# marcros/PartsBasedDetector

Measured on AMD Instinct MI355X. Metric: detections/sec (whole node), person model @640×480, 1/2/4/8 MI355X, higher is better.
Workload: dtype f32

## Files before the change

### partsbaseddetector_amd/csrc/pbd_kernels_dp.hip

```cpp
#include "pbd_device.h"
#include "pbd_dp.h"

#include <math.h>

#include <algorithm>

namespace pbd {

#ifdef PBD_DT_STATS
__device__ unsigned long long g_dt_stats[16];
#define DT_STAT(i)                                                                                      \
    do {                                                                                                \
        const unsigned long long m_ = __ballot(1);                                                      \
        if ((int)__lane_id() == __ffsll((long long)m_) - 1) {                                           \
            atomicAdd(&g_dt_stats[2 * (i)], 1ull);                                                      \
            atomicAdd(&g_dt_stats[2 * (i) + 1], (unsigned long long)__popcll(m_));                      \
        }                                                                                               \
    } while (0)
#else
#define DT_STAT(i)
#endif

template <typename R, bool BZ>
__device__ __forceinline__ R quad_isect(double a, double b, int x0, int x1, R y0f, R y1f)
{
    const double y0 = (double)y0f, y1 = (double)y1f;
    const int dx = x1 - x0;
    const double dd = (double)dx;
    const double sq = (double)(int)__umul24((unsigned)dx, (unsigned)(x1 + x0));
    const double num = BZ ? (y1 - y0) + a * sq : ((y1 - y0) - b * dd) + a * sq;
    return (R)(num / ((2 * a) * dd));
}
template <typename R, bool BZ>
__device__ __forceinline__ R quad_val(double a, double b, int x, R y)
{
    if (BZ) return (R)(a * (double)__mul24(x, x) + (double)y);
    return (R)((a * (double)__mul24(x, x) + b * (double)x) + (double)y);
}

template <typename R> struct StkPairT { R sa, sb, za; unsigned vv; };
static_assert(sizeof(StkPairT<float>) == kStkPairF32 && sizeof(StkPairT<double>) == kStkPairF64, "host sizes the spill stack with these");

#ifndef PBD_DT_CH
#define PBD_DT_CH 16
#endif
constexpr int kDtCH = PBD_DT_CH;
#ifndef PBD_DT_CHC
#define PBD_DT_CHC 16
#endif
constexpr int kDtCHC = PBD_DT_CHC;
#ifndef PBD_DT_RING
#define PBD_DT_RING 8
#endif
constexpr int kDtT = PBD_DT_RING;

template <typename R, bool NARROW>
struct DtRing {
    static constexpr int kSlotBytes = 64 * (2 * (int)sizeof(R) + 4);
    char *zs;
    char *vp;
    StkPairT<R> *g;
    double a, b;
    int lo;
    int tmask, sbytes, soff;
    __device__ __forceinline__ int T() const { return NARROW ? tmask + 1 : kDtT; }
    __device__ __forceinline__ int slot_of(int idx) const { return NARROW ? (idx & tmask) : (idx & (kDtT - 1)); }
    __device__ __forceinline__ int off(int slot) const { return NARROW ? slot * sbytes : slot * kSlotBytes; }
    __device__ __forceinline__ R &z(int slot) { return *reinterpret_cast<R *>(zs + off(slot)); }
    __device__ __forceinline__ R &s(int slot) { return *reinterpret_cast<R *>(zs + off(slot) + (NARROW ? soff : 64 * (int)sizeof(R))); }
    __device__ __forceinline__ int &v(int slot) { return *reinterpret_cast<int *>(vp + off(slot)); }
    __device__ __forceinline__ void push_below(int idx, R zk, R sk, int vk)
    {
        const int slot = slot_of(idx);
        if (idx - lo >= T()) {
            DT_STAT(3);
            const int sl = slot_of(lo);
            g[(size_t)(lo >> 1) * 64] = StkPairT<R>{s(sl), s(sl + 1), z(sl), (unsigned)v(sl) | ((unsigned)v(sl + 1) << 16)};
            lo += 2;
        }
        z(slot) = zk; s(slot) = sk; v(slot) = vk;
    }
    template <bool BZ>
    __device__ __forceinline__ void pop(int idx, R &zk, R &sk, int &vk)
    {
        const int slot = slot_of(idx);
        zk = z(slot); sk = s(slot); vk = v(slot);
        asm volatile("" : "+v"(zk), "+v"(sk), "+v"(vk));
        if (idx < lo) {
            DT_STAT(4);
            const StkPairT<R> e = g[(size_t)((lo - 2) >> 1) * 64];
            const int va = (int)(e.vv & 0xffffu), vb = (int)(e.vv >> 16);
            const int sl = slot_of(lo - 2);
            z(sl) = e.za; s(sl) = e.sa; v(sl) = va;
            sk = e.sb; vk = vb;
            zk = BZ ? quad_isect<R, true>(a, b, va, vb, e.sa, e.sb) : quad_isect<R, false>(a, b, va, vb, e.sa, e.sb);
            lo -= 2;
        }
    }
    static __device__ __forceinline__ DtRing make(char *smem, int lanep, int sh, StkPairT<R> *g, double a, double b)
    {
        const int L = NARROW ? (64 >> sh) : 64;
        return DtRing{smem + lanep * (int)sizeof(R), smem + 2 * L * (int)sizeof(R) + lanep * 4, g, a, b, 0,
                      (kDtT << (NARROW ? sh : 0)) - 1, L * (2 * (int)sizeof(R) + 4), L * (int)sizeof(R)};
    }
};

template <int EPW> __device__ __forceinline__ int dt_get(const int *w, int i)
{
    constexpr int BITS = 32 / EPW;
    return EPW == 1 ? w[i] : (int)(((unsigned)w[i / EPW] >> (BITS * (i % EPW))) & ((1u << BITS) - 1u));
}
template <int EPW> __device__ __forceinline__ void dt_put(int *w, int i, int v)
{
    constexpr int BITS = 32 / EPW;
    if (EPW == 1) w[i] = v;
    else w[i / EPW] |= v << (BITS * (i % EPW));
}

template <typename R, bool BZ, int CH, int EPW, bool NARROW, class LoadChunk, class StoreChunk>
__device__ __forceinline__ void dt_stream(int N, double a, double b, int os0, DtRing<R, NARROW> ring, LoadChunk load, StoreChunk store)
{
    R cur[CH], nxt[CH];
    load(0, cur);
    int k = 0, vk = 0;
    R zk = -RealLimits<R>::inf(), sk = cur[0];
    ring.lo = 0;
    for (int q0 = 0; q0 < N; q0 += CH) {
        if (q0 + CH < N) load(q0 + CH, nxt);
#pragma unroll
        for (int i = 0; i < CH; ++i) {
            const int q = q0 + i;
            if (q >= 1 && q < N) {
                const R sq = cur[i];
                DT_STAT(0);
                R s = quad_isect<R, BZ>(a, b, vk, q, sk, sq);
                while (s <= zk && k > 0) {
                    DT_STAT(1);
                    --k;
                    ring.template pop<BZ>(k, zk, sk, vk);
                    s = quad_isect<R, BZ>(a, b, vk, q, sk, sq);
                }
                ring.push_below(k, zk, sk, vk);
                ++k;
                vk = q; zk = s; sk = sq;
            }
        }
#pragma unroll
        for (int i = 0; i < CH; ++i) cur[i] = nxt[i];
    }
    const int nch = (N + CH - 1) / CH;
    constexpr int NW = CH / EPW;
    for (int cidx = nch - 1; cidx >= 0; --cidx) {
        const int q0 = cidx * CH;
        R out[CH];
        int ptr[NW];
#pragma unroll
        for (int i = 0; i < NW; ++i) ptr[i] = 0;
#pragma unroll
        for (int i = CH - 1; i >= 0; --i) {
            out[i] = (R)0;
            const int q = q0 + i;
            if (q < N) {
                const R osf = (R)(os0 + q);
                DT_STAT(5);
                while (!(zk < osf)) {
                    DT_STAT(2);
                    --k;
                    ring.template pop<BZ>(k, zk, sk, vk);
                }
                out[i] = quad_val<R, BZ>(a, b, os0 + q - vk, sk);
                dt_put<EPW>(ptr, i, vk);
            }
        }
        store(q0, out, ptr);
    }
}

typedef float v4f_u __attribute__((ext_vector_type(4), aligned(4)));
typedef _Float16 v8h_u __attribute__((ext_vector_type(8), aligned(2)));
static_assert(kDtCHC % 8 == 0 && kDtCH % 8 == 0, "int16 pointers and fp16 responses are read 8 at a time");

template <typename R, typename PT> struct DtLine {
    ScoreSrc<R> src;
    int N;
    R *outv; PT *outp;
    int ostr;
    double a, b;
    int os;
    size_t stk;
};
template <typename R, bool RH, typename PT, bool COLS>
__device__ __forceinline__ DtLine<R, PT> dt_line(const DpParams &p, int flat, int j, int fl)
{
    const int l = (COLS ? p.col2level : p.row2level)[flat];
    const LevelDesc d = p.lv[l];
    const int idx = flat - (COLS ? p.coloff : p.rowoff)[l];
    const DtJob job = p.jobs[j];
    const LevelPlanes<DpParams> pl(p, d, p.frame0 + fl, fl);
    const size_t jo = (size_t)j * pl.HW, go = (size_t)job.gm * pl.HW;
    const size_t stk = (size_t)(fl * p.JG + j) * p.stk_per_jf;
    if (COLS) return {{pl.tmp<R>(jo + (size_t)idx * d.rows), nullptr}, d.rows, pl.dt<R>(jo + idx), pl.iy<PT>(go + idx), d.cols,
                      job.ay, job.by, job.osy, stk};
    return {pl.score<R>(job.from_acc, RH, job.plane, (size_t)idx * d.cols), d.cols, pl.tmp<R>(jo + idx), pl.ix<PT>(go + idx), d.rows,
            job.ax, job.bx, job.osx, stk};
}

template <typename R, int CH>
__device__ __forceinline__ void dt_load_chunk(const ScoreSrc<R> &src, int N, int q0, R *buf)
{
    if (src.h) {
        if (q0 + CH <= N) {
#pragma unroll
            for (int v = 0; v < CH / 8; ++v) {
                const v8h_u a0 = *reinterpret_cast<const v8h_u *>(src.h + q0 + 8 * v);
#pragma unroll
                for (int e = 0; e < 8; ++e) buf[8 * v + e] = (R)(float)a0[e];
            }
        } else {
#pragma unroll
            for (int i = 0; i < CH; ++i) buf[i] = (q0 + i < N) ? (R)(float)src.h[q0 + i] : (R)0;
        }
    } else if (sizeof(R) == 4 && q0 + CH <= N) {
        const float *srcf = reinterpret_cast<const float *>(src.v);
#pragma unroll
        for (int v = 0; v < CH / 4; ++v) {
            const v4f_u a0 = *reinterpret_cast<const v4f_u *>(srcf + q0 + 4 * v);
            buf[4 * v] = a0.x; buf[4 * v + 1] = a0.y; buf[4 * v + 2] = a0.z; buf[4 * v + 3] = a0.w;
        }
    } else {
#pragma unroll
        for (int i = 0; i < CH; ++i) buf[i] = (q0 + i < N) ? src.v[q0 + i] : (R)0;
    }
}
template <typename R, typename PT, int CH>
__device__ __forceinline__ void dt_store_chunk(const DtLine<R, PT> &ln, int q0, const R *out, const int *ptr)
{
    R *vp = ln.outv + (size_t)q0 * ln.ostr;
    PT *pp = ln.outp + (size_t)q0 * ln.ostr;
#pragma unroll
    for (int i = 0; i < CH; ++i) {
        if (q0 + i < ln.N) { *vp = out[i]; *pp = (PT)dt_get<4 / (int)sizeof(PT)>(ptr, i); }
        vp += ln.ostr; pp += ln.ostr;
    }
}

template <typename R, bool RH, typename PT, bool BZ, bool NARROW, bool COLS>
__global__ __launch_bounds__(64) __attribute__((amdgpu_waves_per_eu(COLS && sizeof(R) == 4 ? (sizeof(PT) == 1 && !NARROW ? 6 : 5) : 1)))
void k_dt_pass(DpParams p)
{
    constexpr int EPW = 4 / (int)sizeof(PT), CH = COLS ? kDtCHC : kDtCH;
    const int sh = p.lane_shift, lanep = threadIdx.x;
    if (lanep >= (64 >> sh)) return;
    const int wv = (int)blockIdx.z >> sh, lane = (((int)blockIdx.z & ((1 << sh) - 1)) << (6 - sh)) + lanep;
    const int flat = wv * 64 + lane;
    if (flat >= (COLS ? p.ncols_flat : p.nrows_flat)) return;
    const DtLine<R, PT> ln = dt_line<R, RH, PT, COLS>(p, flat, blockIdx.x, blockIdx.y);
    __shared__ __attribute__((aligned(16))) char ring_mem[kDtT * DtRing<R, NARROW>::kSlotBytes];
    DtRing<R, NARROW> ring = DtRing<R, NARROW>::make(ring_mem, lanep, sh, reinterpret_cast<StkPairT<R> *>(p.stk) + ln.stk +
                                                                              (COLS ? p.stk_col_off : p.stk_row_off)[wv] + lane, ln.a, ln.b);
    dt_stream<R, BZ, CH, EPW, NARROW>(ln.N, ln.a, ln.b, ln.os, ring,
                                      [&](int q0, R *buf) { dt_load_chunk<R, CH>(ln.src, ln.N, q0, buf); },
                                      [&](int q0, const R *out, const int *ptr) { dt_store_chunk<R, PT, CH>(ln, q0, out, ptr); });
}

static int dt_lane_shift(const DtOptions &o, long long waves64)
{
    if (o.lane_shift >= 0) return o.lane_shift;
    int sh = 0;
    while (sh < 6 && (waves64 << (sh + 1)) <= 6144) ++sh;
    return sh;
}

template <bool COLS> static void launch_dt_coop(const DpParams &p, int coop_g, int nframes, int nflat, bool bz, hipStream_t s);
static bool dt_coop_fits(int longest);
static int dt_coop_min_shift();

template <class F> static void for_flag(bool b, F &&f) { if (b) f(std::true_type{}); else f(std::false_type{}); }
template <class F> static void for_real(bool f64, F &&f) { if (f64) f(double{}); else f(float{}); }
template <class F> static void for_ptr(bool ptr8, F &&f) { if (ptr8) f(uint8_t{}); else f(int16_t{}); }

template <bool COLS>
static void launch_dt_pass(const DpParams &p0, const DtOptions &o, int nframes, bool f64, hipStream_t s)
{
    const int nflat = COLS ? p0.ncols_flat : p0.nrows_flat;
    if (p0.JG == 0 || nflat == 0) return;
    const int nwv = (nflat + 63) / 64;
    DpParams p = p0;
    p.lane_shift = dt_lane_shift(o, (long long)p.JG * nframes * nwv);
    const bool bz = (COLS ? p.bz_y : p.bz_x) != 0, rh = !COLS && !f64 && p.resp_half;
    if (o.coop && p.lane_shift >= dt_coop_min_shift() && !f64 && !rh && p.ptr8 && dt_coop_fits(p.longest)) {
        launch_dt_coop<COLS>(p, o.coop_g, nframes, nflat, bz, s);
        return;
    }
    const dim3 grid(p.JG, nframes, nwv << p.lane_shift);
    for_ptr(p.ptr8 != 0, [&](auto pt) { for_flag(bz, [&](auto z) {
        using PT = decltype(pt);
        constexpr bool BZ = decltype(z)::value;
        if constexpr (!COLS) {
            if (rh) { PBD_LAUNCH((k_dt_pass<float, true, PT, BZ, false, false>), grid, dim3(64), 0, s, p); return; }
        }
        for_real(f64, [&](auto r) { for_flag(p.lane_shift > 0, [&](auto nw) {
            PBD_LAUNCH((k_dt_pass<decltype(r), false, PT, BZ, decltype(nw)::value, COLS>), grid, dim3(64), 0, s, p);
        }); });
    }); });
}
void launch_dt_rows(const DpParams &p, const DtOptions &o, int nframes, bool f64, hipStream_t s) { launch_dt_pass<false>(p, o, nframes, f64, s); }
void launch_dt_cols(const DpParams &p, const DtOptions &o, int nframes, bool f64, hipStream_t s) { launch_dt_pass<true>(p, o, nframes, f64, s); }

template <bool BZ, typename PT, bool COLS, int G>
__global__ __launch_bounds__(64) void k_dt_coop(DpParams p)
{
    constexpr int kCoopRows = G, kCoopW = 64 / G, kCoopLog = (G == 4 ? 4 : 3);
    static_assert(G == 4 || G == 8, "four or eight rows per wave");
    extern __shared__ __attribute__((aligned(16))) char coop_mem[];
    const int lanep = threadIdx.x, grp = lanep >> kCoopLog, sub = lanep & (kCoopW - 1), gl0 = grp << kCoopLog;
    const int nflat = COLS ? p.ncols_flat : p.nrows_flat;
    const int r = (int)blockIdx.z * kCoopRows + grp;
    const bool active = r < nflat;
    const int rr = active ? r : nflat - 1;
    const DtLine<float, PT> ln = dt_line<float, false, PT, COLS>(p, rr, blockIdx.x, blockIdx.y);
    const int N = active ? ln.N : 0, os0 = ln.os, ostr = ln.ostr;
    const double a = ln.a, b = ln.b;
    const float *src = ln.src.v;
    float *outv = ln.outv;
    PT *outp = ln.outp;
    const int maxn = p.longest;
    float *zs = reinterpret_cast<float *>(coop_mem) + (size_t)grp * 3 * maxn, *ys = zs + maxn;
    int *vs = reinterpret_cast<int *>(ys + maxn);
    int nm = N;
#pragma unroll
    for (int o = kCoopW; o < 64; o <<= 1) nm = max(nm, __shfl_xor(nm, o));
    const int Nmax = __builtin_amdgcn_readfirstlane(nm);
    if (Nmax == 0) return;

    float cur = (sub < N) ? src[sub] : 0.0f;
    float ez = -INFINITY, ey = __shfl(cur, gl0);
    int ev = 0, k = 0, wbase = 0;
    if (sub == 0 && N > 0) { zs[0] = ez; ys[0] = ey; vs[0] = 0; }
    for (int q0 = 0; q0 < Nmax; q0 += kCoopW) {
        const float nxt = (q0 + kCoopW + sub < N) ? src[q0 + kCoopW + sub] : 0.0f;
        for (int i = (q0 == 0 ? 1 : 0); i < kCoopW && q0 + i < Nmax; ++i) {
            const int q = q0 + i;
            const bool rowact = q < N;
            const float yq = __shfl(cur, gl0 + i);
            float s;
            unsigned m;
            for (;;) {
                const int e = wbase + sub;
                s = quad_isect<float, BZ>(a, b, ev, q, ey, yq);
                const bool stay = rowact && e <= k && !((s <= ez) && e > 0);
                m = (unsigned)(__ballot(stay) >> gl0) & ((1u << kCoopW) - 1u);
                const bool lower = rowact && m == 0;
                if (!__any(lower)) break;
                if (lower) { wbase -= kCoopW; k = wbase + kCoopW - 1; ez = zs[wbase + sub]; ey = ys[wbase + sub]; ev = vs[wbase + sub]; }
            }
            const int top = wbase + (rowact ? 31 - __clz((int)m) : 0);
            const float snew = __shfl(s, gl0 + (top & (kCoopW - 1)));
            if (rowact) {
                k = top + 1;
                if ((k & (kCoopW - 1)) == 0) wbase = k;
                if (sub == (k & (kCoopW - 1))) { ev = q; ey = yq; ez = snew; zs[k] = snew; ys[k] = yq; vs[k] = q; }
            }
        }
        cur = nxt;
    }
    for (int p0 = 0; p0 < Nmax; p0 += kCoopW) {
        const int pq = p0 + sub;
        const float osf = (float)(os0 + pq);
        int lo = 0, hi = k;
        while (__any(lo < hi)) {
            const int mid = (lo + hi + 1) >> 1;
            const bool lt = zs[mid] < osf;
            if (lo < hi) { if (lt) lo = mid; else hi = mid - 1; }
        }
        if (pq < N) {
            outv[(size_t)pq * ostr] = quad_val<float, BZ>(a, b, os0 + pq - vs[lo], ys[lo]);
            outp[(size_t)pq * ostr] = (PT)vs[lo];
        }
    }
}

static int dt_coop_min_shift() { return 3; }
static bool dt_coop_fits(int longest)
{
    return (size_t)4 * 3 * longest * sizeof(float) <= (size_t)12 * 1024;
}

template <bool COLS, int G>
static void launch_dt_coop_g(const DpParams &p, int nframes, int nflat, bool bz, hipStream_t s)
{
    dim3 grid(p.JG, nframes, (nflat + G - 1) / G);
    const unsigned lds = (unsigned)((size_t)G * 3 * p.longest * sizeof(float));
    if (bz) PBD_LAUNCH((k_dt_coop<true, uint8_t, COLS, G>), grid, dim3(64), lds, s, p);
    else PBD_LAUNCH((k_dt_coop<false, uint8_t, COLS, G>), grid, dim3(64), lds, s, p);
}
template <bool COLS>
static void launch_dt_coop(const DpParams &p, int coop_g, int nframes, int nflat, bool bz, hipStream_t s)
{
    const long long waves4 = (long long)p.JG * nframes * ((nflat + 3) / 4);
    const bool g8 = coop_g ? coop_g == 8 : (waves4 > 6144 && (size_t)8 * 3 * p.longest * sizeof(float) <= (size_t)12 * 1024);
    if (g8) launch_dt_coop_g<COLS, 8>(p, nframes, nflat, bz, s);
    else launch_dt_coop_g<COLS, 4>(p, nframes, nflat, bz, s);
}

template <typename T, int N> struct CellVec;
#define PBD_CELLVEC(T, E, N) template <> struct CellVec<T, N> { typedef E type __attribute__((ext_vector_type(N), aligned(sizeof(E)))); }
PBD_CELLVEC(float, float, 4); PBD_CELLVEC(float, float, 2); PBD_CELLVEC(double, double, 4); PBD_CELLVEC(double, double, 2);
PBD_CELLVEC(int16_t, short, 4); PBD_CELLVEC(int16_t, short, 2); PBD_CELLVEC(uint8_t, unsigned char, 4); PBD_CELLVEC(uint8_t, unsigned char, 2);
PBD_CELLVEC(_Float16, _Float16, 4); PBD_CELLVEC(_Float16, _Float16, 2);
#undef PBD_CELLVEC

template <typename T, int kCpt>
__device__ __forceinline__ void load_cells(const T *src, int n, T *dst)
{
    if (n == kCpt) {
        const typename CellVec<T, kCpt>::type v = *reinterpret_cast<const typename CellVec<T, kCpt>::type *>(src);
#pragma unroll
        for (int e = 0; e < kCpt; ++e) dst[e] = (T)v[e];
    } else {
#pragma unroll
        for (int e = 0; e < kCpt; ++e) dst[e] = (e < n) ? src[e] : (T)0;
    }
}
template <typename T, int kCpt>
__device__ __forceinline__ void load_cells_wide(const T *src, T *dst)
{
    const typename CellVec<T, kCpt>::type v = *reinterpret_cast<const typename CellVec<T, kCpt>::type *>(src);
#pragma unroll
    for (int e = 0; e < kCpt; ++e) dst[e] = (T)v[e];
}
template <typename T, int kCpt>
__device__ __forceinline__ void store_cells(T *dst, int n, const T *src)
{
    if (n == kCpt) {
        typename CellVec<T, kCpt>::type v;
#pragma unroll
        for (int e = 0; e < kCpt; ++e) v[e] = src[e];
        *reinterpret_cast<typename CellVec<T, kCpt>::type *>(dst) = v;
    } else {
#pragma unroll
        for (int e = 0; e < kCpt; ++e) if (e < n) dst[e] = src[e];
    }
}

template <typename R, int kCpt, int MAXM, bool RH>
__global__ __launch_bounds__(256) __attribute__((amdgpu_waves_per_eu(MAXM <= 6 && sizeof(R) == 4 ? 4 : 1)))
void k_dp_combine(DpParams p)
{
    constexpr int SUB = 4 / kCpt;
    const long long gidx = (long long)blockIdx.x * blockDim.x + threadIdx.x;
    const long long qidx = gidx / SUB;
    if (qidx >= p.quad_per_frame) return;
    const int fl = blockIdx.z, frame = p.frame0 + fl;
    const CombineJob cj = p.cjobs[blockIdx.y];
    const LevelDesc d = p.lv[level_of<&LevelDesc::quad_off>(p.lv, 0, p.nlevels, qidx)];
    const int HWi = d.rows * d.cols;
    const size_t HW = (size_t)HWi;
    const int local = (int)(qidx - d.quad_off) * 4 + (int)(gidx % SUB) * kCpt;
    if (local >= HWi) return;
    const int n = min(kCpt, HWi - local);
    const LevelPlanes<DpParams> pl(p, d, frame, fl);
    const R *dtp = pl.dt<R>();
    uint8_t *ik = pl.Ik(local);
    R accv[MAXM][kCpt];
#pragma unroll
    for (int pm = 0; pm < MAXM; ++pm) {
#pragma unroll
        for (int e = 0; e < kCpt; ++e) accv[pm][e] = (R)0;
        if (pm < cj.npar) {
            const ScoreSrc<R> rs = pl.score<R>(false, RH, cj.filter[pm], local);
            if constexpr (RH) {
                _Float16 hv[kCpt];
                load_cells<_Float16, kCpt>(rs.h, n, hv);
#pragma unroll
                for (int e = 0; e < kCpt; ++e) accv[pm][e] = (R)(float)hv[e];
            } else {
                load_cells<R, kCpt>(rs.v, n, accv[pm]);
            }
        }
    }
    const int __attribute__((address_space(4))) *childs = (const int __attribute__((address_space(4))) *)p.childs;
    constexpr int kChildInts = 3 + kMaxMix;
    static_assert(sizeof(ChildDesc) == kChildInts * sizeof(int), "ChildDesc is read as 3 + kMaxMix ints");
    const float __attribute__((address_space(4))) *biasw = (const float __attribute__((address_space(4))) *)p.biasw;
    for (int ch = cj.child_begin; ch < cj.child_end; ++ch) {
        ChildDesc cd;
        {
            const int __attribute__((address_space(4))) *ci = childs + (size_t)ch * kChildInts;
            cd.job_begin = ci[0]; cd.nmix = ci[1]; cd.slot = ci[2];
#pragma unroll
            for (int k = 0; k < MAXM; ++k) cd.bias_off[k] = ci[3 + k];
        }
        const R *dtc = dtp + (size_t)cd.job_begin * HW;
        float bw[MAXM][MAXM];
#pragma unroll
        for (int mm = 0; mm < MAXM; ++mm)
#pragma unroll
            for (int pm = 0; pm < MAXM; ++pm)
                bw[mm][pm] = (mm < cd.nmix && pm < cj.npar) ? biasw[cd.bias_off[mm] + pm] : 0.0f;
        R dtv[MAXM][kCpt];
#pragma unroll
        for (int mm = 0; mm < MAXM; ++mm) {
#pragma unroll
            for (int e = 0; e < kCpt; ++e) dtv[mm][e] = -RealLimits<R>::inf();
            if (mm < cd.nmix) load_cells_wide<R, kCpt>(dtc + (size_t)mm * HW + local, dtv[mm]);
        }
#pragma unroll
        for (int pm = 0; pm < MAXM; ++pm) {
            if (pm < cj.npar) {
                uint8_t oik[kCpt];
                R best[kCpt];
                int bi[kCpt];
#pragma unroll
                for (int e = 0; e < kCpt; ++e) bi[e] = 0;
                if (cd.nmix == 1) {
#pragma unroll
                    for (int e = 0; e < kCpt; ++e) best[e] = dtv[0][e] + (R)bw[0][pm];
                } else {
#pragma unroll
                    for (int e = 0; e < kCpt; ++e) {
                        best[e] = -RealLimits<R>::inf();
#pragma unroll
                        for (int mm = 0; mm < MAXM; ++mm) pick_max<R>(dtv[mm][e] + (R)bw[mm][pm], mm, best[e], bi[e]);
                    }
                }
#pragma unroll
                for (int e = 0; e < kCpt; ++e) {
                    oik[e] = (uint8_t)bi[e];
                    accv[pm][e] = accv[pm][e] + best[e];
                }
                store_cells<uint8_t, kCpt>(ik + (size_t)(cd.slot + pm) * HW, n, oik);
            }
        }
    }
    R *acc = pl.acc<R>(local);
#pragma unroll
    for (int pm = 0; pm < MAXM; ++pm)
        if (pm < cj.npar) store_cells<R, kCpt>(acc + (size_t)(cj.acc_plane + pm) * HW, n, accv[pm]);
}

void launch_dp_combine(const DpParams &p, int ncjobs, int nframes, bool f64, hipStream_t s)
{
    if (ncjobs == 0 || p.quad_per_frame == 0) return;
    const dim3 g2((unsigned)((p.quad_per_frame * 2 + 255) / 256), ncjobs, nframes), g4((unsigned)((p.quad_per_frame + 255) / 256), ncjobs, nframes);
    auto launch = [&](auto m) {
        constexpr int M = decltype(m)::value;
        if (f64) PBD_LAUNCH((k_dp_combine<double, 2, M, false>), g2, dim3(256), 0, s, p);
        else if (p.resp_half) PBD_LAUNCH((k_dp_combine<float, 4, M, true>), g4, dim3(256), 0, s, p);
        else PBD_LAUNCH((k_dp_combine<float, 4, M, false>), g4, dim3(256), 0, s, p);
    };
    if (p.max_mix <= 2) launch(std::integral_constant<int, 2>{});
    else if (p.max_mix <= 4) launch(std::integral_constant<int, 4>{});
    else if (p.max_mix <= 6) launch(std::integral_constant<int, 6>{});
    else if (p.max_mix <= 8) launch(std::integral_constant<int, 8>{});
    else launch(std::integral_constant<int, 16>{});
}

template <typename R>
__global__ __launch_bounds__(256) void k_dp_combine_seq(DpParams p)
{
    const long long idx = (long long)blockIdx.x * blockDim.x + threadIdx.x;
    if (idx >= p.cell_per_frame) return;
    const int fl = blockIdx.z;
    const SeqCombineJob sj = p.sjobs[blockIdx.y];
    const LevelDesc d = p.lv[level_of(p.lv, 0, p.nlevels, idx)];
    const size_t local = (size_t)(idx - d.cell_off);
    const LevelPlanes<DpParams> pl(p, d, p.frame0 + fl, fl);
    const size_t HW = pl.HW;
    const R *dtp = pl.dt<R>((size_t)sj.job_begin * HW + local);
    R dtv[kMaxMix];
    for (int mm = 0; mm < sj.nmix; ++mm) dtv[mm] = dtp[(size_t)mm * HW];
    for (int pm = 0; pm < sj.npar; ++pm) {
        int bi;
        const R best = reduce_max<R>(sj.nmix, [&](int mm) { return dtv[mm] + (R)p.biasw[sj.bias_off[mm] + pm]; }, bi);
        *pl.Ik((size_t)(sj.slot + pm) * HW + local) = (uint8_t)bi;
        R *t = pl.acc<R>((size_t)sj.target[pm] * HW + local);
        const R base = !sj.init[pm] ? *t : pl.score<R>(false, sizeof(R) == 4 && p.resp_half, sj.filter[pm], local)[0];
        *t = base + best;
    }
}

void launch_dp_combine_seq(const DpParams &p, int nsjobs, int nframes, bool f64, hipStream_t s)
{
    if (nsjobs == 0 || p.cell_per_frame == 0) return;
    dim3 grid((unsigned)((p.cell_per_frame + 255) / 256), nsjobs, nframes);
    for_real(f64, [&](auto r) { PBD_LAUNCH(k_dp_combine_seq<decltype(r)>, grid, dim3(256), 0, s, p); });
}

template <typename R>
__global__ __launch_bounds__(256) void k_dp_root(DpParams p)
{
    const long long idx = (long long)blockIdx.x * blockDim.x + threadIdx.x;
    if (idx >= p.cell_per_frame) return;
    const int c = blockIdx.y, fl = blockIdx.z, frame = p.frame0 + fl;
    const RootJob rj = p.rjobs[c];
    const LevelDesc d = p.lv[level_of(p.lv, 0, p.nlevels, idx)];
    const size_t local = (size_t)(idx - d.cell_off);
    const LevelPlanes<DpParams> pl(p, d, frame);
    const bool rh = sizeof(R) == 4 && p.resp_half;
    int bi;
    const R best = reduce_max<R>(rj.nmix, [&](int mm) { return pl.score<R>((rj.from_acc >> mm) & 1, rh, rj.plane[mm], local)[0] + (R)rj.bias; }, bi);
    const size_t o = (size_t)c * pl.HW + local;
    *pl.rootv<R>(o) = best;
    *pl.rooti(o) = bi;
}

void launch_dp_root(const DpParams &p, int nframes, bool f64, hipStream_t s)
{
    if (p.cell_per_frame == 0) return;
    dim3 grid((unsigned)((p.cell_per_frame + 255) / 256), p.NC, nframes);
    for_real(f64, [&](auto r) { PBD_LAUNCH(k_dp_root<decltype(r)>, grid, dim3(256), 0, s, p); });
}

constexpr int kFindEPT = 4, kFindBlock = 256, kFindSpan = kFindEPT * kFindBlock;

template <typename R>
__device__ __forceinline__ int find_hits(const ArgminParams &p, long long base, bool hit[kFindEPT])
{
    const R *rv = static_cast<const R *>(p.rootv);
    int c = 0;
#pragma unroll
    for (int e = 0; e < kFindEPT; ++e) {
        const long long o = base + e;
        hit[e] = o < p.ntotal && rv[o] > (R)p.thresh;
        if (p.root_max) hit[e] = hit[e] && p.root_max[o];
        c += hit[e] ? 1 : 0;
    }
    return c;
}

template <typename R>
__global__ __launch_bounds__(kFindBlock) void k_argmin_count(ArgminParams p)
{
    bool hit[kFindEPT];
    const int c = find_hits<R>(p, (long long)blockIdx.x * kFindSpan + threadIdx.x * kFindEPT, hit);
    __shared__ int wsum[kFindBlock / 64];
    const int lane = threadIdx.x & 63, incl = wave_incl_scan(c);
    if (lane == 63) wsum[threadIdx.x >> 6] = incl;
    __syncthreads();
    if (threadIdx.x == 0) {
        int t = 0;
#pragma unroll
        for (int w = 0; w < kFindBlock / 64; ++w) t += wsum[w];
        p.blk[blockIdx.x] = t;
    }
}

__global__ __launch_bounds__(1024) void k_argmin_scan(ArgminParams p)
{
    __shared__ int wsum[16];
    __shared__ int carry_s;
    if (threadIdx.x == 0) carry_s = 0;
    __syncthreads();
    const int lane = threadIdx.x & 63, w = threadIdx.x >> 6;
    for (int b0 = 0; b0 < p.nblk; b0 += 1024) {
        const int b = b0 + threadIdx.x;
        const int v = b < p.nblk ? p.blk[b] : 0;
        const int incl = wave_incl_scan(v);
        if (lane == 63) wsum[w] = incl;
        __syncthreads();
        int off = carry_s;
        for (int k = 0; k < w; ++k) off += wsum[k];
        if (b < p.nblk) p.blk[b] = off + incl - v;
        __syncthreads();
        if (threadIdx.x == 1023) carry_s = off + incl;
        __syncthreads();
    }
    if (threadIdx.x == 0) p.payload[0] = carry_s;
}

template <typename R>
__global__ __launch_bounds__(kFindBlock) void k_argmin_emit(ArgminParams p)
{
    bool hit[kFindEPT];
    const long long base = (long long)blockIdx.x * kFindSpan + threadIdx.x * kFindEPT;
    const int c = find_hits<R>(p, base, hit);
    __shared__ int wsum[kFindBlock / 64];
    const int lane = threadIdx.x & 63, w = threadIdx.x >> 6, incl = wave_incl_scan(c);
    if (lane == 63) wsum[w] = incl;
    __syncthreads();
    if (c == 0) return;
    int slot = p.blk[blockIdx.x] + incl - c;
    for (int k = 0; k < w; ++k) slot += wsum[k];
    const long long per_frame = p.cell_per_frame * p.NC;
#pragma unroll
    for (int e = 0; e < kFindEPT; ++e) {
        if (!hit[e]) continue;
        const int mine = slot++;
        if (mine >= p.capacity) continue;
        const long long o = base + e;
        const int frame = (int)(o / per_frame);
        root_record(p.payload + 1 + (size_t)mine * p.stride, p.lv, 0, p.nlevels, p.NC, frame, o - (long long)frame * per_frame,
                    static_cast<const R *>(p.rootv)[o], p.rooti[o]);
    }
}

void launch_argmin_find(const ArgminParams &p, bool f64, hipStream_t s)
{
    for_real(f64, [&](auto r) { PBD_LAUNCH(k_argmin_count<decltype(r)>, dim3(p.nblk), dim3(kFindBlock), 0, s, p); });
    PBD_LAUNCH(k_argmin_scan, dim3(1), dim3(1024), 0, s, p);
    for_real(f64, [&](auto r) { PBD_LAUNCH(k_argmin_emit<decltype(r)>, dim3(p.nblk), dim3(kFindBlock), 0, s, p); });
}
int argmin_find_span() { return kFindSpan; }

template <typename R, typename PT>
__global__ __launch_bounds__(64) void k_argmin_walk(ArgminParams p)
{
    __shared__ int visited[kWalkMaxParts][64];
    __shared__ uint8_t visited_m[kWalkMaxParts][64];
    const int ncand = min(p.payload[0], p.capacity);
    for (int i = blockIdx.x * blockDim.x + threadIdx.x; i < ncand; i += gridDim.x * blockDim.x) {
    int32_t *rec = p.payload + 1 + (size_t)i * p.stride;
    const int frame = rec[0], c = rec[1], l = rec[2];
    const LevelDesc d = p.lv[l];
    const LevelPlanes<ArgminParams> pl(p, d, frame);
    const R scale = (R)p.scales[l];
    const PartWalk *walk = p.walk + p.walk_off[c];
    const int nparts = p.walk_off[c + 1] - p.walk_off[c];
    int32_t *rects = rec + 8;
    for (int pidx = 0; pidx < nparts; ++pidx) {
        int x, y, m;
        if (pidx == 0) {
            x = rec[3]; y = rec[4]; m = rec[7];
        } else {
            const PartWalk w = walk[pidx];
            const int par = visited[w.parent][threadIdx.x];
            const WalkPos ch = walk_child<PT>(pl, w, par & 0xffff, par >> 16, visited_m[w.parent][threadIdx.x], p.walk_mode == PBD_WALK_ARGMAX);
            x = ch.x; y = ch.y; m = ch.m;
        }
        visited[pidx][threadIdx.x] = x | (y << 16);
        visited_m[pidx][threadIdx.x] = (uint8_t)m;
        const PartRect r = part_rect<R>(x, y, walk[pidx].ksize[m], scale);
        rects[pidx * 4 + 0] = r.x1;
        rects[pidx * 4 + 1] = r.y1;
        rects[pidx * 4 + 2] = r.x2 - r.x1;
        rects[pidx * 4 + 3] = r.y2 - r.y1;
    }
    rec[0] = frame + p.frame_offset;
    if (p.lv_frame) {
        rec[0] = p.lv_frame[l] + p.frame_offset;
        rec[2] = p.lv_local[l];
    }
    rec[6] = nparts;
    rec[7] = 0;
    }
}

void launch_argmin_walk(const ArgminParams &p, bool f64, hipStream_t s)
{
    const int blocks = std::max(std::min((p.capacity + 63) / 64, 2048), 1);
    for_real(f64, [&](auto r) { for_ptr(p.ptr8 != 0, [&](auto pt) {
        PBD_LAUNCH((k_argmin_walk<decltype(r), decltype(pt)>), dim3(blocks), dim3(64), 0, s, p);
    }); });
}

}

#ifdef PBD_DT_STATS
extern "C" int pbd_debug_dt_stats(unsigned long long *out, int reset)
{
    if (out && hipMemcpyFromSymbol(out, HIP_SYMBOL(pbd::g_dt_stats), sizeof(pbd::g_dt_stats)) != hipSuccess) return -1;
    if (reset) {
        unsigned long long z[16] = {0};
        if (hipMemcpyToSymbol(HIP_SYMBOL(pbd::g_dt_stats), z, sizeof(z)) != hipSuccess) return -1;
    }
    return 0;
}
#endif
```

Before: 1096.

## Batch ring spills and reloads across the wavefront with high/low watermarks

```diff
diff --git a/partsbaseddetector_amd/csrc/pbd_kernels_dp.hip b/partsbaseddetector_amd/csrc/pbd_kernels_dp.hip
--- a/partsbaseddetector_amd/csrc/pbd_kernels_dp.hip
+++ b/partsbaseddetector_amd/csrc/pbd_kernels_dp.hip
@@ -53,6 +53,20 @@
 #define PBD_DT_RING 8
 #endif
 constexpr int kDtT = PBD_DT_RING;
+#ifndef PBD_DT_HIGH
+#define PBD_DT_HIGH 6
+#endif
+#ifndef PBD_DT_LOW
+#define PBD_DT_LOW 2
+#endif
+#ifndef PBD_DT_LOW_RO
+#define PBD_DT_LOW_RO 6
+#endif
+constexpr int kDtHigh = PBD_DT_HIGH;
+constexpr int kDtLow = PBD_DT_LOW;
+constexpr int kDtLowRO = PBD_DT_LOW_RO;
+static_assert(kDtHigh >= 3 && kDtHigh <= kDtT + 1, "a spilling lane has its oldest pair in the ring; a lane over the ring always spills");
+static_assert(kDtLow <= kDtT - 2 && kDtLowRO <= kDtT - 2, "a pair is only reloaded into a ring with room for two entries");
 
 template <typename R, bool NARROW>
 struct DtRing {
@@ -69,16 +83,38 @@
     __device__ __forceinline__ R &z(int slot) { return *reinterpret_cast<R *>(zs + off(slot)); }
     __device__ __forceinline__ R &s(int slot) { return *reinterpret_cast<R *>(zs + off(slot) + (NARROW ? soff : 64 * (int)sizeof(R))); }
     __device__ __forceinline__ int &v(int slot) { return *reinterpret_cast<int *>(vp + off(slot)); }
+    __device__ __forceinline__ int high() const { return T() - (kDtT - kDtHigh); }
+    __device__ __forceinline__ int low_readout() const { return kDtLowRO < 0 ? -1 : T() - (kDtT - kDtLowRO); }
     __device__ __forceinline__ void push_below(int idx, R zk, R sk, int vk)
     {
         const int slot = slot_of(idx);
-        if (idx - lo >= T()) {
-            DT_STAT(3);
-            const int sl = slot_of(lo);
-            g[(size_t)(lo >> 1) * 64] = StkPairT<R>{s(sl), s(sl + 1), z(sl), (unsigned)v(sl) | ((unsigned)v(sl + 1) << 16)};
-            lo += 2;
+        const int n = idx - lo + 1;
+        if (__any(n > T())) {
+            if (n >= high()) {
+                DT_STAT(3);
+                const int sl = slot_of(lo);
+                g[(size_t)(lo >> 1) * 64] = StkPairT<R>{s(sl), s(sl + 1), z(sl), (unsigned)v(sl) | ((unsigned)v(sl + 1) << 16)};
+                lo += 2;
+            }
         }
         z(slot) = zk; s(slot) = sk; v(slot) = vk;
+    }
+    template <bool BZ>
+    __device__ __forceinline__ void service_reload(int k, int drained, int low)
+    {
+        const int n = k - lo;
+        if (__any(n <= drained && lo > 0)) {
+            if (n <= low && lo > 0) {
+                DT_STAT(7);
+                const StkPairT<R> e = g[(size_t)((lo - 2) >> 1) * 64];
+                const int va = (int)(e.vv & 0xffffu), vb = (int)(e.vv >> 16);
+                const int sl = slot_of(lo - 2);
+                z(sl) = e.za; s(sl) = e.sa; v(sl) = va;
+                z(sl + 1) = BZ ? quad_isect<R, true>(a, b, va, vb, e.sa, e.sb) : quad_isect<R, false>(a, b, va, vb, e.sa, e.sb);
+                s(sl + 1) = e.sb; v(sl + 1) = vb;
+                lo -= 2;
+            }
+        }
     }
     template <bool BZ>
     __device__ __forceinline__ void pop(int idx, R &zk, R &sk, int &vk)
@@ -133,6 +169,7 @@
             if (q >= 1 && q < N) {
                 const R sq = cur[i];
                 DT_STAT(0);
+                ring.template service_reload<BZ>(k, 1, kDtLow);
                 R s = quad_isect<R, BZ>(a, b, vk, q, sk, sq);
                 while (s <= zk && k > 0) {
                     DT_STAT(1);
@@ -163,6 +200,7 @@
             if (q < N) {
                 const R osf = (R)(os0 + q);
                 DT_STAT(5);
+                ring.template service_reload<BZ>(k, 0, ring.low_readout());
                 while (!(zk < osf)) {
                     DT_STAT(2);
                     --k;
```

Result: faster. 1136 (median of 6 runs) (+3.7%).
